# chriscoey/Hypatia.jl

Measured on AMD Instinct MI355X. Metric: IPM iterations/sec (+ ms per KKT solve): dense n=5000, PosSemidefTri side 200 (Float64, QRCholDense + CombinedStepper), higher is better.
Workload: dtype f64

## Files before the change

hypatia.jl_amd/csrc/capi.hip:

```cpp
#include <unistd.h>
#include "../../include/hypatia_hip.h"
#include "syssolver.hpp"
#include <chrono>
#include <cstring>

using namespace hyp;

struct hyp_ctx { Ctx c; hyp_ctx(int d) : c(d) {} };
struct hyp_cone { hyp_ctx* ctx; Cone* cone; };
struct hyp_sys { hyp_ctx* ctx; SysSolver* s; };
struct hyp_symindef { hyp_ctx* ctx; SymIndefSys* s; };
struct hyp_comm { hyp_ctx* ctx; void* nccl; int nranks, rank; };
namespace hyp {
struct QrcpFact;
QrcpFact* qrcp_create(Ctx& c, int m, int n, const double* hA, int lda, const double* hb);
void qrcp_get(QrcpFact* f, int* jpvt, double* R, double* rdiag, double* qtb);
void qrcp_apply_q(QrcpFact* f, bool trans, double* hx);
void qrcp_destroy(QrcpFact* f);
}
struct hyp_qrcp { hyp_ctx* ctx; hyp::QrcpFact* f; };

namespace hyp {
void rccl_allreduce_inplace(void* comm, double* d_buf, long count, int op, hipStream_t st);
void rccl_unique_id(char* out128);
// ... 488 lines not shown
  sys->ctx->c.sync();
  sys->ctx->c.timers[6] += now_s() - t0;
  API_END(sys->ctx)
}
int hyp_sys_lhs_export_dev(hyp_sys* sys, void* dst_device) {
  API_BEGIN
  Ctx& c = sys->ctx->c;
  c.d2d(dst_device, sys->s->lhs.p, (size_t)sys->s->nmp * sys->s->nmp * sizeof(double));
  c.sync();
  API_END(sys->ctx)
}
int hyp_sys_lhs_import_dev(hyp_sys* sys, const void* src_device) {
  API_BEGIN
  Ctx& c = sys->ctx->c;
  c.d2d(sys->s->lhs.p, src_device, (size_t)sys->s->nmp * sys->s->nmp * sizeof(double));
  c.sync();
  API_END(sys->ctx)
}
int hyp_sys_set_lhs(hyp_sys* sys, const double* in) {
  API_BEGIN
  Ctx& c = sys->ctx->c;
  c.h2d(sys->s->lhs.p, in, (size_t)sys->s->nmp * sys->s->nmp * sizeof(double));
  c.sync();
  API_END(sys->ctx)
}
int hyp_sys_potrs(hyp_sys* sys, double* x) {
  API_BEGIN
  Ctx& c = sys->ctx->c;
  SysSolver* s = sys->s;
  HYP_REQUIRE(s->fact_ok, "potrs: no valid factorization");
  c.h2d(s->tmpn.p, x, (size_t)s->nmp * sizeof(double));
  s->potrs(s->tmpn.d());
  c.d2h(x, s->tmpn.p, (size_t)s->nmp * sizeof(double));
  c.sync();
  API_END(sys->ctx)
}
int hyp_sys_solve3(hyp_sys* sys, double* sol_vec, const double* rhs_vec) {
// ... 686 lines not shown
```

hypatia.jl_amd/csrc/directions_multi.hip:

```cpp
#include <cstring>
#include "syssolver.hpp"
#include <chrono>

namespace hyp {

void seg_dots(Ctx& c, int B, int len, const double* a, const double* b, int off, int stride, double* out);
constexpr int MR = 2;

template <int NR, int TPB, int U>
__global__ __launch_bounds__(TPB) void gemv_t_multi_kernel(int m, double alpha, const double* __restrict__ A, long lda,
                                                           const double* __restrict__ X, long ldx, double beta, double* __restrict__ Y,
                                                           long ldy) {
  constexpr int NW = TPB / 64;
  __shared__ double red[NR][NW];
  const int col = blockIdx.x;
  const double* a = A + (long)col * lda;
  double s[NR][2 * U];
#pragma unroll
  for (int r = 0; r < NR; ++r)
#pragma unroll
    for (int u = 0; u < 2 * U; ++u) s[r][u] = 0.0;
  int i = 0;
  typedef double d2_t __attribute__((ext_vector_type(2)));
  const bool wide = (((uintptr_t)a | (uintptr_t)X | ((uintptr_t)ldx * sizeof(double))) & 15) == 0;
// ... 1386 lines not shown
  const auto t0 = std::chrono::steady_clock::now();
  const double tau = h_point[it], kap = h_point[ik];
  m_rhs.ensure((size_t)(MR + 1) * dv * d);
  v_tmp.ensure((size_t)MR * dv * d);
  const bool resident = resident_flow;
  if (!resident) {
    if (nmp > 0) update_lhs_fact(info, used_fallback);
    if (use_sqrt_out)
      for (size_t k = 0; k < cones.size(); ++k) use_sqrt_out[k] = use_sqrt[k];
    if (*info != 0) { ctx.sync(); return; }
    step_directions_rest(false, tau, kap, tau_residual, mu, max_ref_steps, res_norm_cutoff, min_impr_tol, h_dirs, res_norms, n_solves,
                         h_sol_const, hs_const, hs_dirs, false, nullptr, nullptr);
    last_update_lhs_s = last_rest_update_lhs_s + std::chrono::duration<double>(t_rest0 - t0).count();
    return;
  }
  assemble_lhs();
  factor_lhs_begin();
  if (upload_after) {
    hs_point = ctx.stage_host((size_t)dv + 2 * (size_t)it + 2 * (size_t)MR * dv);
    hs_res = hs_point + dv;
    hs_const = hs_res + it;
    hs_dirs = hs_const + it;
    upload(ctx.stream);
  }
  if (upload_late) {
    hs_point = ctx.stage_host((size_t)dv + 2 * (size_t)it + 2 * (size_t)MR * dv);
    hs_res = hs_point + dv;
    hs_const = hs_res + it;
    hs_dirs = hs_const + it;
    HYP_CHECK(hipStreamWaitEvent(ctx.stream2, up_ev0, 0));
    upload(ctx.stream2);
// ... 149 lines not shown
```

hypatia.jl_amd/csrc/gemm_f64.hpp:

```cpp
#pragma once
#include <hip/hip_runtime.h>
#include <stdint.h>

namespace hyp {

typedef double d4_t __attribute__((ext_vector_type(4)));

enum GemmTri : int {
  GEMM_FULL = 0,
  GEMM_UPPER = 1,
  GEMM_UPPER_RECT = 2,
};

enum GemmKRange : int {
  KR_ALL = 0,
  KR_LE_M = 1,
  KR_GE_M = 2,
  KR_LE_N = 3,
  KR_GE_N = 4,
};

struct GemmArgs {
  int M, N, K;
  const double* A; long lda; long strideA;
// ... 4 lines not shown
  int krange;
  int batch;
  int tiles_m, tiles_n;
  int cm_blk; long cm_stride;
  int tile_hint;
  int epi;
  int tag;
  int hiprio;
  int tri_off;
  int splitk_req;
  int splitk; int kchunk; double* part; long part_ld; long part_stride;
  int vec2;
  const int* tile_map;
  int splitk_base, tail_q, tail_first, tail_chunk;
  int* tile_cnt;
};

struct GemmScratch {
  double* splitk_ws = nullptr;
  size_t splitk_ws_bytes = 0;
  int* tile_map = nullptr;
  int tile_map_T = -1;
  int* tile_cnt = nullptr;
  long tile_cnt_n = 0;
  struct TrapMap { int tiles_m = 0, tiles_n = 0, tri_off = 0; long nblk = 0; int* map = nullptr; unsigned long used = 0; };
  TrapMap trap[16];
  unsigned long trap_clock = 0;
  void release() {
    for (TrapMap& t : trap) { if (t.map) (void)hipFree(t.map); t = TrapMap(); }
    if (splitk_ws) (void)hipFree(splitk_ws);
    if (tile_map) (void)hipFree(tile_map);
    if (tile_cnt) (void)hipFree(tile_cnt);
    splitk_ws = nullptr; splitk_ws_bytes = 0; tile_map = nullptr; tile_map_T = -1; tile_cnt = nullptr; tile_cnt_n = 0;
  }
};

hipError_t gemm_f64_launch(hipStream_t st, bool transa, GemmArgs a, GemmScratch* scratch = nullptr);
hipError_t schur_syrk_cols(hipStream_t st, GemmArgs a, int c0, int c1, GemmScratch* scratch);
hipError_t schur_syrk_edge(hipStream_t st, const GemmArgs& a, int* N0);

}
```

hypatia.jl_amd/csrc/gemm_f64_kernel.hpp:

```cpp
#pragma once
#include "gemm_f64.hpp"
#include <vector>

namespace hyp {

#ifdef HYP_GEMM_PROBE
__device__ unsigned long long gemm_probe_acc[8];
#define GEMM_PROBE_T(x) const unsigned long long x = __builtin_amdgcn_s_memtime()
#else
#define GEMM_PROBE_T(x)
#endif

constexpr int BK = 16, LDS_S = BK + 2;
typedef const volatile double __attribute__((address_space(3))) lds_cv_f64;
constexpr int GEMM_THREADS = 256;

__device__ __forceinline__ void upper_tile_from_linear(int idx, int& tm, int& tn) {
  int t = (int)((sqrt(8.0 * (double)idx + 1.0) - 1.0) * 0.5);
  while ((long)(t + 1) * (t + 2) / 2 <= idx) ++t;
  while ((long)t * (t + 1) / 2 > idx) --t;
  tn = t;
  tm = idx - t * (t + 1) / 2;
}

// ... 317 lines not shown
                                     double alpha, double beta, double* __restrict__ C, long ldc, int S_extra, int tail_first,
                                     const int* __restrict__ tile_rank, int T, long part_batch, long strideC) {
  const int m = blockIdx.x * blockDim.x + threadIdx.x;
  const int n = blockIdx.y;
  if (m >= M || (upper && m > n + tri_off)) return;
  part += (long)blockIdx.z * part_batch;
  C += (long)blockIdx.z * strideC;
  double s = 0.0;
  for (int z = 0; z < S; ++z) s += part[(long)z * part_stride + (long)n * part_ld + m];
  if (S_extra > 0 && tile_rank[(m >> 7) + (n >> 7) * T] >= tail_first)
    for (int z = S; z < S + S_extra; ++z) s += part[(long)z * part_stride + (long)n * part_ld + m];
  double* cp = C + (long)n * ldc + m;
  *cp = alpha * s + (beta != 0.0 ? beta * (*cp) : 0.0);
}

static const int* upper_tile_map(GemmScratch& gs, int T, long nblk) {
  if (gs.tile_map_T == T) return gs.tile_map;
  std::vector<int> logical;
  logical.reserve(2 * nblk);
  const int ST = 8, nst = (T + ST - 1) / ST;
  for (int J = 0; J < nst; ++J)
    for (int I = 0; I <= J; ++I)
      for (int j = 0; j < ST; ++j)
        for (int i = 0; i < ST; ++i) {
          const int tm = I * ST + i, tn = J * ST + j;
          if (tm < T && tn < T && tm <= tn) { logical.push_back(tm); logical.push_back(tn); }
        }
  std::vector<int> hw(2 * nblk + (size_t)T * T, -1);
  const long q = nblk / 8, r = nblk % 8;
  for (long b = 0; b < nblk; ++b) {
// ... 39 lines not shown
    hw[2 * b] = logical[2 * L];
    hw[2 * b + 1] = logical[2 * L + 1];
    hw[2 * nblk + hw[2 * b] + (size_t)hw[2 * b + 1] * tiles_m] = (int)b;
  }
  if (slot->map) { (void)hipDeviceSynchronize(); (void)hipFree(slot->map); }
  *slot = GemmScratch::TrapMap();
  int* d = nullptr;
  if (hipMalloc((void**)&d, hw.size() * sizeof(int)) != hipSuccess) return nullptr;
  if (hipMemcpy(d, hw.data(), hw.size() * sizeof(int), hipMemcpyHostToDevice) != hipSuccess) { (void)hipFree(d); return nullptr; }
  slot->map = d; slot->tiles_m = tiles_m; slot->tiles_n = tiles_n; slot->tri_off = tri_off; slot->nblk = nblk; slot->used = ++gs.trap_clock;
  *nblk_out = nblk;
  return d;
}

template <int CB, int R>
__global__ __launch_bounds__(256) void syrk_edge_kernel(int K, int N, int N0, int e0, int r, const double* __restrict__ A, long lda, double alpha,
                                                        double beta, double* __restrict__ C, long ldc) {
  typedef double d2_t __attribute__((ext_vector_type(2)));
  __shared__ double red[CB][R][4];
  const int i0 = blockIdx.x * CB;
  const double* a[CB];
  const double* x[R];
#pragma unroll
  for (int c = 0; c < CB; ++c) a[c] = A + (long)min(i0 + c, N - 1) * lda;
#pragma unroll
  for (int e = 0; e < R; ++e) x[e] = A + (long)min(N0 + e0 + e, N - 1) * lda;
  constexpr int NS = (CB * R <= 32) ? 2 : 1;
  double s[CB][R][NS];
#pragma unroll
  for (int c = 0; c < CB; ++c)
#pragma unroll
    for (int e = 0; e < R; ++e)
#pragma unroll
      for (int h = 0; h < NS; ++h) s[c][e][h] = 0.0;
  const int nfull = K / 512;
// ... 28 lines not shown
#pragma unroll
    for (int e = 0; e < R; ++e) {
      double t = (NS == 2) ? s[c][e][0] + s[c][e][NS - 1] : s[c][e][0];
#pragma unroll
      for (int off = 32; off > 0; off >>= 1) t += __shfl_down(t, off);
      if ((threadIdx.x & 63) == 0) red[c][e][threadIdx.x >> 6] = t;
    }
  __syncthreads();
  if (threadIdx.x < CB * R) {
    const int c = threadIdx.x / R, e = threadIdx.x % R;
    const int i = i0 + c, col = N0 + e0 + e;
    if (i < N && e0 + e < r && i <= col) {
      const double t = (red[c][e][0] + red[c][e][1]) + (red[c][e][2] + red[c][e][3]);
      double* dst = C + (long)col * ldc + i;
      *dst = alpha * t + (beta != 0.0 ? beta * (*dst) : 0.0);
    }
  }
}

static bool syrk_edge_ok(const GemmArgs& a) {
  static const bool edge_on = [] { const char* e = getenv("HYP_SYRK_EDGE"); return !(e && atoi(e) == 0); }();
  return edge_on && ((uintptr_t)a.A % 16 == 0) && (a.lda % 2 == 0);
}
static hipError_t syrk_edge_launch(hipStream_t st, const GemmArgs& a, int N0, int r) {
  static const int cb_env = [] { const char* e = getenv("HYP_SYRK_EDGE_CB"); return e ? atoi(e) : 8; }();
  const int cb = cb_env;
  for (int e0 = 0; e0 < r; e0 += 8) {
    if (cb == 8) hipLaunchKernelGGL((syrk_edge_kernel<8, 8>), dim3((a.N + 7) / 8), dim3(256), 0, st, a.K, a.N, N0, e0, r, a.A, a.lda, a.alpha, a.beta, a.C, a.ldc);
    else hipLaunchKernelGGL((syrk_edge_kernel<4, 8>), dim3((a.N + 3) / 4), dim3(256), 0, st, a.K, a.N, N0, e0, r, a.A, a.lda, a.alpha, a.beta, a.C, a.ldc);
  }
  return hipGetLastError();
}

hipError_t gemm_f64_launch(hipStream_t st, bool transa, GemmArgs a, GemmScratch* gs) {
  if (a.M <= 0 || a.N <= 0 || a.batch <= 0) return hipSuccess;
  if (a.tag == 1 && transa && a.tri == GEMM_UPPER && a.A == a.B && a.lda == a.ldb && a.batch == 1 && a.epi == 0 &&
      a.krange == KR_ALL && a.M == a.N && a.N >= 1024 && a.N % 128 != 0 && a.N % 128 <= 32 && a.K >= 4096) {
    const int r = a.N % 128, N0 = a.N - r;
    GemmArgs m = a;
    m.M = m.N = N0;
    hipError_t e = gemm_f64_launch(st, transa, m, gs);
    if (e != hipSuccess) return e;
    GemmArgs s = a;
    s.tag = 0; s.M = a.N; s.N = r;
    s.B = a.A + (long)N0 * a.lda;
    s.C = a.C + (long)N0 * a.ldc;
    s.tri = GEMM_UPPER_RECT; s.tri_off = N0;
    s.tile_hint = 64; s.splitk_req = 8;
    if (syrk_edge_ok(a)) return syrk_edge_launch(st, a, N0, r);
    return gemm_f64_launch(st, transa, s, gs);
  }
  const long t128 = (long)((a.M + 127) / 128) * ((a.N + 127) / 128) * a.batch;
  const bool small = (a.tile_hint == 64) || (a.tile_hint == 0 && t128 < 192);
  const int BT = small ? 64 : 128;
  a.tiles_m = (a.M + BT - 1) / BT;
  a.tiles_n = (a.N + BT - 1) / BT;
  long nblk;
  const int* trap_map = nullptr;
  static const bool trap_on = [] { const char* e = getenv("HYP_GEMM_TRAP_MAP"); return !(e && atoi(e) == 0); }();
  if (a.tri == GEMM_UPPER) {
    int T = a.tiles_n;
    nblk = (long)T * (T + 1) / 2;
  } else {
    nblk = (long)a.tiles_m * a.tiles_n;
    if (trap_on && gs && a.tag == 1 && transa && a.tri == GEMM_UPPER_RECT && !small && a.batch == 1 && a.epi == 0 && a.krange == KR_ALL && nblk >= 64) {
// ... 85 lines not shown
      gs->tile_cnt = nullptr; gs->tile_cnt_n = 0;
      if (hipMalloc((void**)&gs->tile_cnt, (size_t)nblk * sizeof(int)) == hipSuccess && hipMemset(gs->tile_cnt, 0, (size_t)nblk * sizeof(int)) == hipSuccess)
        gs->tile_cnt_n = nblk;
    }
    if (gs->tile_cnt_n >= nblk) a.tile_cnt = gs->tile_cnt;
  }
  if (a.tag == 1 && transa && !small) {
    hipLaunchKernelGGL((gemm_f64_kernel<true, 4, 1>), grid, dim3(GEMM_THREADS), 0, st, a);
  } else if (transa) {
    if (small) hipLaunchKernelGGL((gemm_f64_kernel<true, 2, 0>), grid, dim3(GEMM_THREADS), 0, st, a);
    else hipLaunchKernelGGL((gemm_f64_kernel<true, 4, 0>), grid, dim3(GEMM_THREADS), 0, st, a);
  } else {
    if (small) hipLaunchKernelGGL((gemm_f64_kernel<false, 2, 0>), grid, dim3(GEMM_THREADS), 0, st, a);
    else hipLaunchKernelGGL((gemm_f64_kernel<false, 4, 0>), grid, dim3(GEMM_THREADS), 0, st, a);
  }
  if (a.splitk > 1 && a.tile_cnt == nullptr)
    hipLaunchKernelGGL(splitk_reduce_kernel, dim3((a.M + 255) / 256, a.N, a.batch), dim3(256), 0, st, a.M, a.N, a.tri != GEMM_FULL ? 1 : 0, a.tri_off,
                       a.splitk_base, a.part, a.part_ld, a.part_stride, a.alpha, a.beta, a.C, a.ldc, a.tail_q - 1, a.tail_first,
                       a.tile_map ? a.tile_map + 2 * nblk : nullptr, trap_map ? a.tiles_m : a.tiles_n, (long)a.splitk * a.part_stride, a.strideC);
  return hipGetLastError();
}

hipError_t schur_syrk_cols(hipStream_t st, GemmArgs a, int c0, int c1, GemmScratch* gs) {
  static const int s_env = [] { const char* e = getenv("HYP_CHOL_SPLIT_S"); return e ? atoi(e) : 0; }();
  if (c0 == 0) {
    GemmArgs l = a;
    l.M = l.N = c1;
    if (s_env > 0) l.splitk_req = s_env;
    return gemm_f64_launch(st, true, l, gs);
  }
  const int N = a.N;
  int r = N % 128, N0 = N - r;
  if (!(r > 0 && r <= 32 && a.K >= 4096 && syrk_edge_ok(a))) { r = 0; N0 = N; }
  GemmArgs t = a;
  t.M = N0; t.N = N0 - c0;
  t.B = a.A + (long)c0 * a.lda;
  t.C = a.C + (long)c0 * a.ldc;
  t.tri = GEMM_UPPER_RECT; t.tri_off = c0;
  if (t.N > 0) {
    const long tm = (t.M + 127) / 128, tn = (t.N + 127) / 128, tc0 = c0 / 128;
    long real = 0;
    for (long j = 0; j < tn; ++j) real += std::min(tm, tc0 + j + 1);
    int S = 1;
    double best = 1e30;
    const double eps = ((double)t.M * t.N * 4.6e-12) / (2.6e-7 * a.K);
    for (int q = 1; q <= 8; ++q) {
      if (a.K / q < 1024) break;
      const double cost = (double)((real * q + 511) / 512) / q + (q > 1 ? q * eps : 0.0);
      if (cost < best - 1e-9) { best = cost; S = q; }
    }
    if (s_env > 0) S = s_env;
    t.splitk_req = S;
    hipError_t e = gemm_f64_launch(st, true, t, gs);
    if (e != hipSuccess) return e;
  }
  if (r > 0) return syrk_edge_launch(st, a, N0, r);
  return hipSuccess;
}

hipError_t schur_syrk_edge(hipStream_t st, const GemmArgs& a, int* N0) {
  const int r = a.N % 128;
  *N0 = a.N;
  if (!(r > 0 && r <= 32 && a.N >= 1024 && a.K >= 4096 && a.M == a.N && syrk_edge_ok(a))) return hipSuccess;
  *N0 = a.N - r;
  return syrk_edge_launch(st, a, *N0, r);
}

}
// ... 1 lines not shown
```

hypatia.jl_amd/csrc/syssolver.hip:

```cpp
#include <cstring>
#include "syssolver.hpp"
#include <chrono>

namespace hyp {

__global__ void increase_diag_kernel(int n, double* A, long lda) {
  const int j = blockIdx.x * blockDim.x + threadIdx.x;
  if (j < n) {
    const double d = A[(long)j * lda + j];
    A[(long)j * lda + j] = (1.0 + 1e-5) * fmax(d, 1000 * 2.220446049250313e-16);
  }
}

SysSolver::SysSolver(Ctx& c, int n_, int p_, int q_, const std::vector<Cone*>& cs) : ctx(c), n(n_), p(p_), q(q_), nmp(n_ - p_), cones(cs) {
  HYP_REQUIRE(n >= 0 && p >= 0 && q >= 0 && p <= n, "sys: sizes");
  offs.assign(cones.size() + 1, 0);
  for (size_t k = 0; k < cones.size(); ++k) offs[k + 1] = offs[k] + cones[k]->dim;
  HYP_REQUIRE(offs.back() == q, "sys: cone dimensions do not sum to q");
  use_sqrt.assign(cones.size(), 0);
  make_psd_runs();
  const size_t d = sizeof(double);
  G.alloc((size_t)q * n * d);
  if (p > 0) {
    GQ1.alloc((size_t)q * p * d);
// ... 12 lines not shown
  tmpn.alloc((size_t)std::max(n, 1) * d);
  Gx.alloc((size_t)std::max(q, 1) * d);
  HGx.alloc((size_t)std::max(q, 1) * d);
  tmpq.alloc((size_t)std::max(q, 1) * d);
  sol.alloc((size_t)(n + p + q + 1) * d);
  rhs.alloc((size_t)(n + p + q + 1) * d);
}

SysSolver::~SysSolver() {
  if (const char* e = getenv("HYP_RP_PREFETCH_STATS"))
    if (e[0] == '1') fprintf(stderr, "[residual_products prefetch] handed out %ld, recomputed %ld\n", rp_pre_hits, rp_pre_misses);
  if (const char* e = getenv("HYP_SHP_PRELAUNCH_STATS"))
    if (e[0] == '1') fprintf(stderr, "[sqrt_hess_prod prelaunch] used %ld, not used %ld\n", shp_used, shp_unused);
  if (const char* e = getenv("HYP_CHOL_SPLIT_STATS"))
    if (e[0] == '1') fprintf(stderr, "[chol split] %ld factorizations in two column groups\n", chol_split_count);
  if (rp_pre_host) (void)hipHostFree(rp_pre_host);
  for (hipEvent_t e : {rp_pre_ev, plan_ev_fork, plan_ev_done, dirs_copied_ev, up_ev0, up_ev1, split_ev_ready, split_ev_done, ov_ev_fork})
    if (e) (void)hipEventDestroy(e);
}

void SysSolver::make_psd_runs() {
  static const bool on = [] { const char* e = getenv("HYP_PSD_GROUP"); return !(e && e[0] == '0'); }();
  if (!on) return;
  size_t k = 0;
  while (k < cones.size()) {
    PsdCone* pk = (cones[k]->kind == CONE_PSD) ? static_cast<PsdCone*>(cones[k]) : nullptr;
    size_t e = k + 1;
    if (pk)
      while (e < cones.size() && cones[e]->kind == CONE_PSD && static_cast<PsdCone*>(cones[e])->side == pk->side) ++e;
    const int cnt = (int)(e - k);
// ... 338 lines not shown
void SysSolver::comm_times_flush() {
  for (const CommEv& e : comm_ev_pending) {
    HYP_CHECK(hipEventSynchronize(e.b));
    float ms = 0;
    HYP_CHECK(hipEventElapsedTime(&ms, e.a, e.b));
    comm_ms[e.site] += ms;
    comm_ev_free.push_back(e.a);
    comm_ev_free.push_back(e.b);
  }
  comm_ev_pending.clear();
}

void SysSolver::allreduce_lhs() {
  const bool have = (comm_fn != nullptr || rccl_comm != nullptr);
  if (!have || (ks_world <= 1 && !dist())) return;
  const int kw = ks_world;
  ks_world = 1;
  hipEvent_t ev_whole = nullptr;
  comm_time_begin(14, &ev_whole);
  try {
    const long cnt = (long)nmp * (nmp + 1) / 2;
    lhs_tri.ensure((size_t)cnt * sizeof(double));
    const dim3 grid((nmp + 255) / 256, nmp);
    hipLaunchKernelGGL(tri_pack_kernel, grid, dim3(256), 0, ctx.stream, nmp, lhs.d(), (long)nmp, lhs_tri.d(), 0);
    allreduce_dev(lhs_tri.d(), cnt, 0, 0);
    hipLaunchKernelGGL(tri_pack_kernel, grid, dim3(256), 0, ctx.stream, nmp, lhs.d(), (long)nmp, lhs_tri.d(), 1);
    HYP_CHECK(hipGetLastError());
  } catch (...) {
    ks_world = kw;
    throw;
// ... 200 lines not shown
}

void SysSolver::block_hess_prod_vec(double* d_out, const double* d_in) {
  for (size_t k = 0; k < cones.size(); ++k) {
    Cone* ck = cones[k];
    if (const int used = run_hess_prod(k, d_out + offs[k], q, d_in + offs[k], q, 1)) { k += used - 1; continue; }
    if (ck->use_dual_barrier) ck->inv_hess_prod(d_out + offs[k], q, d_in + offs[k], q, 1);
    else ck->hess_prod(d_out + offs[k], q, d_in + offs[k], q, 1);
  }
}

void SysSolver::update_lhs_fact(int* info, int* used_fallback) {
  *info = 0;
  *used_fallback = 0;
  if (nmp == 0) return;
  assemble_lhs();
  factor_lhs(info, used_fallback);
}

static bool force_bk_env();

void SysSolver::prelaunch_sqrt_hess() {
  static const bool on = [] { const char* e = getenv("HYP_SHP_PRELAUNCH"); return e && e[0] == '1'; }();
  shp_prelaunched = false;
  if (!on || shp_wasted >= 2 || nmp <= 0 || p != 0 || dist() || ks_world > 1 || !dirs_resident() || force_bk_env() ||
      ctx.stream != ctx.stream_primary)
    return;
  {
    const char* ff = getenv("HYP_FORCE_FACT_FAIL");
    if (ff && ff[0] && ff[0] != '0') return;
  }
// ... 6 lines not shown
  if (!all_sqrt) return;
  const double* gq2 = GQ2();
  HYP_CHECK(hipEventRecord(ctx.ev[0], ctx.stream));
  int idx = 0;
  for (size_t k = 0; k < cones.size(); ++k) {
    Cone* ck = cones[k];
    if (ck->use_dual_barrier) ck->inv_sqrt_hess_prod(HGQ2.d() + idx, q, gq2 + offs[k], q, nmp);
    else ck->sqrt_hess_prod(HGQ2.d() + idx, q, gq2 + offs[k], q, nmp);
    idx += ck->dim;
  }
  HYP_CHECK(hipEventRecord(ctx.ev[1], ctx.stream));
  shp_prelaunched = true;
  shp_epoch = ctx.cone_epoch;
}

void SysSolver::assemble_lhs() {
  if (split_unjoined) {
    HYP_CHECK(hipStreamWaitEvent(ctx.stream, split_ev_done, 0));
    split_unjoined = false;
  }
  chol_split_n1 = 0;
  const bool pre = shp_prelaunched && shp_epoch == ctx.cone_epoch && nmp > 0 && !dist() && ks_world == 1;
  if (shp_prelaunched) {
    if (pre) { shp_wasted = 0; ++shp_used; }
    else { ++shp_wasted; ++shp_unused; }
  }
  shp_prelaunched = false;
  if (!pre) group_inverses();
  if (nmp == 0) return;
  const double* gq2 = GQ2();
  if (!pre)
// ... 31 lines not shown
    if (!pre) HYP_CHECK(hipEventRecord(ctx.ev[1], ctx.stream));
    GemmArgs s{};
    long r0 = 0, r1 = idx;
    if (ks_world > 1) {
      const long per = (((long)idx + ks_world - 1) / ks_world + 15) / 16 * 16;
      r0 = std::min<long>((long)idx, per * ks_rank);
      r1 = std::min<long>((long)idx, r0 + per);
    }
    if (use_ov && assemble_lhs_overlapped(r0, r1, ov_groups)) {
      HYP_CHECK(hipEventRecord(ctx.ev[2], ctx.stream));
      ctx.kstat[4] += 1;
      return;
    }
    s.M = nmp; s.N = nmp; s.K = (int)(r1 - r0); s.A = HGQ2.d() + r0; s.lda = q; s.B = HGQ2.d() + r0; s.ldb = q; s.C = lhs.d(); s.ldc = nmp;
    s.alpha = 1; s.beta = 0; s.tri = GEMM_UPPER; s.krange = KR_ALL; s.batch = 1; s.tag = 1;
    {
      bool all_sqrt = true;
      for (int v : use_sqrt) all_sqrt &= (v != 0);
      const int n1 = chol_split_point(nmp, s.K);
      if (n1 > 0 && all_sqrt && !dist() && ks_world == 1 && !force_bk_env() && ctx.stream == ctx.stream_primary) {
        if (!split_ev_ready) {
          HYP_CHECK(hipEventCreateWithFlags(&split_ev_ready, hipEventDisableTiming));
          HYP_CHECK(hipEventCreateWithFlags(&split_ev_done, hipEventDisableTiming));
        }
        schur_split_begin(ctx, nmp, s.K, s.A, q, lhs.d(), lhs_fact.d(), n1, d_info.i(), ctx.lane(2).s, split_ev_ready, split_ev_done);
        chol_split_n1 = n1;
        split_unjoined = true;
        HYP_CHECK(hipEventRecord(ctx.ev[2], ctx.stream));
        ctx.kstat[4] += 1;
        return;
      }
    }
    gemm(ctx, true, s);
    HYP_CHECK(hipEventRecord(ctx.ev[2], ctx.stream));
    ctx.kstat[4] += 1;
  } else {
    ctx.zero(lhs.p, (size_t)nmp * nmp * sizeof(double));
  }
  for (size_t k = 0; k < cones.size(); ++k) {
    if (use_sqrt[k]) continue;
    Cone* ck = cones[k];
    double* prod_k = HGQ2.d() + offs[k];
    if (ck->use_dual_barrier) ck->inv_hess_prod(prod_k, q, gq2 + offs[k], q, nmp);
    else ck->hess_prod(prod_k, q, gq2 + offs[k], q, nmp);
    long r0 = 0, r1 = ck->dim;
    if (ks_world > 1) {
      const long per = (((long)ck->dim + ks_world - 1) / ks_world + 15) / 16 * 16;
      r0 = std::min<long>((long)ck->dim, per * ks_rank);
      r1 = std::min<long>((long)ck->dim, r0 + per);
    }
    if (r1 <= r0) continue;
    GemmArgs g{};
    g.M = nmp; g.N = nmp; g.K = (int)(r1 - r0); g.A = gq2 + offs[k] + r0; g.lda = q; g.B = prod_k + r0; g.ldb = q; g.C = lhs.d(); g.ldc = nmp;
    g.alpha = 1; g.beta = 1; g.tri = GEMM_UPPER; g.krange = KR_ALL; g.batch = 1;
    gemm(ctx, true, g);
  }
  allreduce_lhs();
}

static bool force_bk_env() {
  const char* fb = getenv("HYP_FORCE_BK");
  return fb && fb[0] && fb[0] != '0';
}

int SysSolver::chol_split_point(int n, int K) {
  static const int pct = [] { const char* e = getenv("HYP_CHOL_SPLIT"); return e ? atoi(e) : 0; }();
  static const int min_n = [] { const char* e = getenv("HYP_CHOL_SPLIT_MIN_N"); return e ? atoi(e) : 3072; }();
  if (pct <= 0 || n < min_n || K < 4096) return 0;
  int n1 = (int)((long)n * std::min(pct, 95) / 100) / 128 * 128;
  return potrf_split_ok(n, n1) ? n1 : 0;
}

void SysSolver::factor_lhs_begin() {
  if (nmp == 0 || force_bk_env()) return;
  use_bk = false;
  if (chol_split_n1 > 0) {
    HYP_CHECK(hipEventRecord(ctx.ev[3], ctx.stream));
    schur_split_finish(ctx, nmp, lhs.d(), lhs_fact.d(), chol_split_n1, dinv.d(), d_info.i(), split_ev_done);
    chol_split_n1 = 0;
    split_unjoined = false;
    ++chol_split_count;
  } else {
    ctx.d2d(lhs_fact.p, lhs.p, (size_t)nmp * nmp * sizeof(double));
    HYP_CHECK(hipEventRecord(ctx.ev[3], ctx.stream));
    potrf_upper_batched(ctx, nmp, lhs_fact.d(), nmp, 0, 1, dinv.d(), d_info.i());
  }
  HYP_CHECK(hipEventRecord(ctx.ev[4], ctx.stream));
  ctx.d2h(ctx.h_info + Ctx::H_INFO_FACT, d_info.p, sizeof(int));
  tri.invalidate();
  if (ctx.trsv_plan_sb(nmp) <= 0) return;
  static const bool plan_lane = [] { const char* e = getenv("HYP_PLAN_LANE"); return e && e[0] == '1'; }();
  if (plan_lane && Ctx::max_lanes() >= 3 && ctx.stream == ctx.stream_primary) {
    if (!plan_ev_fork) {
      HYP_CHECK(hipEventCreateWithFlags(&plan_ev_fork, hipEventDisableTiming));
      HYP_CHECK(hipEventCreateWithFlags(&plan_ev_done, hipEventDisableTiming));
    }
    HYP_CHECK(hipEventRecord(plan_ev_fork, ctx.stream));
    {
// ... 25 lines not shown
void SysSolver::factor_lhs_end(int* info, int* used_fallback, bool times_later) {
  *info = 0;
  *used_fallback = 0;
  if (nmp == 0) return;
  const bool force_bk = force_bk_env();
  use_bk = false;
  join_plan();
  if (!force_bk) {
    *info = ctx.h_info[Ctx::H_INFO_FACT];
    if (!times_later) factor_lhs_times();
  }
  if (force_bk || *info != 0) {
    use_bk = true;
    *used_fallback = 1;
    const int chol_info = force_bk ? 0 : *info;
    ctx.d2d(lhs_fact.p, lhs.p, (size_t)nmp * nmp * sizeof(double));
    *info = bk_after_failed_cholesky(ctx, bk, nmp, lhs_fact.d(), nmp, dinv.d(), d_info.i(), chol_info, lhs.d(), nmp);
    if (*info != 0) {
      *used_fallback = 2;
      ctx.d2d(lhs_fact.p, lhs.p, (size_t)nmp * nmp * sizeof(double));
      hipLaunchKernelGGL(increase_diag_kernel, dim3((nmp + 255) / 256), dim3(256), 0, ctx.stream, nmp, lhs_fact.d(), (long)nmp);
      *info = bk.factor(ctx, nmp, lhs_fact.d(), nmp, dinv.d());
    }
  }
  {
    const char* ff = getenv("HYP_FORCE_FACT_FAIL");
    if (ff && ff[0] && ff[0] != '0') *info = 1;
  }
  fact_ok = (*info == 0);
  if (use_bk || !fact_ok) tri.invalidate();
// ... 1284 lines not shown
```

hypatia.jl_amd/csrc/syssolver.hpp:

```cpp
#pragma once
#include <chrono>
#include "cones.hpp"

namespace hyp {

void dev_sub_absmax(Ctx& c, int n, double* a, const double* b, double* d_out);
void dev_sub_absmax_cols(Ctx& c, int n, int nr, double* a, const double* b, long ld, double* d_out, double* work);

struct SysSolver {
  Ctx& ctx;
  int n, p, q, nmp;
  std::vector<Cone*> cones;
  std::vector<int> offs;
  DBuf G;
  DBuf GQ1;
  DBuf GQ2s;
  DBuf Qm;
  DBuf Rinv;
  DBuf HGQ2;
  DBuf lhs;
  DBuf lhs_tri;
  DBuf lhs_fact, dinv, d_info;
  TriSolvePlan tri;
  DBuf QpbxGHbz, Gx, HGx, GQ1x, HGQ1x, tmpn, sol, rhs, tmpq;
// ... 10 lines not shown
  void run_dder3(const PsdRun& r, const double* d_dir, double* d_out);
  void run_prox_launch(const PsdRun& r, double irtmu, double* d_out);
  DBuf prox_scal;
  BKFact bk;
  bool use_bk = false;
  DBuf bk_work;

  SysSolver(Ctx& c, int n_, int p_, int q_, const std::vector<Cone*>& cs);
  ~SysSolver();
  SysSolver(const SysSolver&) = delete;
  SysSolver& operator=(const SysSolver&) = delete;
  const double* GQ2() const { return p == 0 ? G.d() : GQ2s.d(); }
  void load(const double* hG, const double* hGQ1, const double* hGQ2, const double* hQ, const double* hR);
  void block_hess_prod_vec(double* d_out, const double* d_in);
  void update_lhs_fact(int* info, int* used_fallback);
  void assemble_lhs();
  void factor_lhs(int* info, int* used_fallback);
  void prelaunch_sqrt_hess();
  bool shp_prelaunched = false;
  unsigned long shp_epoch = 0;
  int shp_wasted = 0;
  long shp_used = 0, shp_unused = 0;
  int chol_split_point(int n, int K);
  int chol_split_n1 = 0;
  long chol_split_count = 0;
  bool split_unjoined = false;
  hipEvent_t split_ev_ready = nullptr, split_ev_done = nullptr;
  hipEvent_t ov_ev_fork = nullptr;
  void factor_lhs_begin();
  void factor_lhs_end(int* info, int* used_fallback, bool times_later = false);
  hipEvent_t plan_ev_fork = nullptr, plan_ev_done = nullptr;
// ... 163 lines not shown
```

Measured before the change: 58.50.

## Write Schur product directly into factor buffer and fuse edge SYRK into split-K finish

The split-K reduction for the upper-triangular Schur complement SYRK now writes its result to both lhs and lhs_fact, so the full nmp×nmp device-to-device copy before Cholesky can be skipped when the lower part of lhs_fact is known to be valid. The edge-column SYRK for the N%128 remainder is folded into the same finish kernel launch instead of running as separate kernels. State flags track when lhs_fact is filled and invalidate that on imports, allreduce, split factorization or fallback paths. This adds a second store stream in the reduce and more bookkeeping that must stay correct across code paths.

```diff
diff --git a/hypatia.jl_amd/csrc/capi.hip b/hypatia.jl_amd/csrc/capi.hip
--- a/hypatia.jl_amd/csrc/capi.hip
+++ b/hypatia.jl_amd/csrc/capi.hip
@@ -526,6 +526,7 @@
   API_BEGIN
   Ctx& c = sys->ctx->c;
   c.d2d(sys->s->lhs.p, src_device, (size_t)sys->s->nmp * sys->s->nmp * sizeof(double));
+  sys->s->lhs_fact_filled = false; sys->s->lhs_fact_lower_ok = false;
   c.sync();
   API_END(sys->ctx)
 }
@@ -533,6 +534,7 @@
   API_BEGIN
   Ctx& c = sys->ctx->c;
   c.h2d(sys->s->lhs.p, in, (size_t)sys->s->nmp * sys->s->nmp * sizeof(double));
+  sys->s->lhs_fact_filled = false; sys->s->lhs_fact_lower_ok = false;
   c.sync();
   API_END(sys->ctx)
 }
diff --git a/hypatia.jl_amd/csrc/directions_multi.hip b/hypatia.jl_amd/csrc/directions_multi.hip
--- a/hypatia.jl_amd/csrc/directions_multi.hip
+++ b/hypatia.jl_amd/csrc/directions_multi.hip
@@ -1424,7 +1424,7 @@
     last_update_lhs_s = last_rest_update_lhs_s + std::chrono::duration<double>(t_rest0 - t0).count();
     return;
   }
-  assemble_lhs();
+  assemble_lhs(true);
   factor_lhs_begin();
   if (upload_after) {
     hs_point = ctx.stage_host((size_t)dv + 2 * (size_t)it + 2 * (size_t)MR * dv);
diff --git a/hypatia.jl_amd/csrc/gemm_f64.hpp b/hypatia.jl_amd/csrc/gemm_f64.hpp
--- a/hypatia.jl_amd/csrc/gemm_f64.hpp
+++ b/hypatia.jl_amd/csrc/gemm_f64.hpp
@@ -42,6 +42,7 @@
   const int* tile_map;
   int splitk_base, tail_q, tail_first, tail_chunk;
   int* tile_cnt;
+  double* C2; long ldc2;
 };
 
 struct GemmScratch {
@@ -54,6 +55,7 @@
   struct TrapMap { int tiles_m = 0, tiles_n = 0, tri_off = 0; long nblk = 0; int* map = nullptr; unsigned long used = 0; };
   TrapMap trap[16];
   unsigned long trap_clock = 0;
+  bool c2_done = false;
   void release() {
     for (TrapMap& t : trap) { if (t.map) (void)hipFree(t.map); t = TrapMap(); }
     if (splitk_ws) (void)hipFree(splitk_ws);
diff --git a/hypatia.jl_amd/csrc/gemm_f64_kernel.hpp b/hypatia.jl_amd/csrc/gemm_f64_kernel.hpp
--- a/hypatia.jl_amd/csrc/gemm_f64_kernel.hpp
+++ b/hypatia.jl_amd/csrc/gemm_f64_kernel.hpp
@@ -355,6 +355,81 @@
   *cp = alpha * s + (beta != 0.0 ? beta * (*cp) : 0.0);
 }
 
+struct SchurFinishArgs {
+  int M, N, tri_off, S_extra, tail_first, T;
+  const double* part; long part_ld, part_stride;
+  const int* tile_rank;
+  double alpha, beta;
+  double* C; long ldc;
+  double* C2; long ldc2;
+  int n_edge, K, r;
+  const double* A; long lda;
+};
+
+template <int S, int ROWS>
+__device__ __forceinline__ void schur_reduce_body(const SchurFinishArgs& p, int b) {
+  typedef double d2_t __attribute__((ext_vector_type(2)));
+  constexpr int TPC = 128 / ROWS;
+  constexpr int CPP = 256 / TPC;
+  constexpr int U = 2;
+  int tm, tn;
+  upper_tile_from_linear(b >> 3, tm, tn);
+  const int extra = (p.S_extra > 0 && p.tile_rank[tm + tn * p.T] >= p.tail_first) ? p.S_extra : 0;
+  const int m = tm * 128 + ROWS * ((int)threadIdx.x % TPC);
+  const int nb = tn * 128 + (b & 7) * 16 + (int)threadIdx.x / TPC;
+#pragma unroll 1
+  for (int c = 0; c < 16; c += U * CPP) {
+    bool ok[U][ROWS];
+    long off[U];
+    double v[U][S][ROWS], cold[U][ROWS];
+#pragma unroll
+    for (int u = 0; u < U; ++u) {
+      const int n = nb + c + u * CPP;
+#pragma unroll
+      for (int h = 0; h < ROWS; ++h) ok[u][h] = (n < p.N) && (m + h < p.M) && (m + h <= n + p.tri_off);
+      off[u] = ok[u][0] ? (long)n * p.part_ld + m : 0;
+#pragma unroll
+      for (int z = 0; z < S; ++z) {
+        const double* src = p.part + (long)z * p.part_stride + off[u];
+        if (ROWS == 2) {
+          const d2_t t = *reinterpret_cast<const d2_t*>(src);
+          v[u][z][0] = t.x; v[u][z][ROWS - 1] = t.y;
+        } else {
+          v[u][z][0] = *src;
+        }
+      }
+      if (p.beta != 0.0) {
+        const double* cp = p.C + (ok[u][0] ? (long)n * p.ldc + m : 0);
+#pragma unroll
+        for (int h = 0; h < ROWS; ++h) cold[u][h] = cp[h];
+      }
+    }
+#pragma unroll
+    for (int u = 0; u < U; ++u) {
+      const int n = nb + c + u * CPP;
+      double res[ROWS];
+#pragma unroll
+      for (int h = 0; h < ROWS; ++h) {
+        double s = 0.0;
+#pragma unroll
+        for (int z = 0; z < S; ++z) s += v[u][z][h];
+        for (int z = S; z < S + extra; ++z) s += p.part[(long)z * p.part_stride + off[u] + h];
+        res[h] = p.alpha * s + (p.beta != 0.0 ? p.beta * cold[u][h] : 0.0);
+      }
+      if (!ok[u][0]) continue;
+      double* cp = p.C + (long)n * p.ldc + m;
+      double* cp2 = p.C2 ? p.C2 + (long)n * p.ldc2 + m : nullptr;
+      if (ROWS == 2 && ok[u][ROWS - 1]) {
+        *reinterpret_cast<d2_t*>(cp) = (d2_t){res[0], res[ROWS - 1]};
+        if (cp2) *reinterpret_cast<d2_t*>(cp2) = (d2_t){res[0], res[ROWS - 1]};
+      } else {
+        *cp = res[0];
+        if (cp2) *cp2 = res[0];
+      }
+    }
+  }
+}
+
 static const int* upper_tile_map(GemmScratch& gs, int T, long nblk) {
   if (gs.tile_map_T == T) return gs.tile_map;
   std::vector<int> logical;
@@ -424,11 +499,10 @@
 }
 
 template <int CB, int R>
-__global__ __launch_bounds__(256) void syrk_edge_kernel(int K, int N, int N0, int e0, int r, const double* __restrict__ A, long lda, double alpha,
-                                                        double beta, double* __restrict__ C, long ldc) {
+__device__ __forceinline__ void syrk_edge_body(int i0, int K, int N, int N0, int e0, int r, const double* __restrict__ A, long lda, double alpha,
+                                               double beta, double* __restrict__ C, long ldc, double* __restrict__ C2, long ldc2) {
   typedef double d2_t __attribute__((ext_vector_type(2)));
   __shared__ double red[CB][R][4];
-  const int i0 = blockIdx.x * CB;
   const double* a[CB];
   const double* x[R];
 #pragma unroll
@@ -487,41 +561,94 @@
       const double t = (red[c][e][0] + red[c][e][1]) + (red[c][e][2] + red[c][e][3]);
       double* dst = C + (long)col * ldc + i;
       *dst = alpha * t + (beta != 0.0 ? beta * (*dst) : 0.0);
-    }
-  }
+      if (C2) C2[(long)col * ldc2 + i] = *dst;
+    }
+  }
+}
+
+template <int CB, int R>
+__global__ __launch_bounds__(256) void syrk_edge_kernel(int K, int N, int N0, int e0, int r, const double* __restrict__ A, long lda, double alpha,
+                                                        double beta, double* __restrict__ C, long ldc, double* __restrict__ C2, long ldc2) {
+  syrk_edge_body<CB, R>(blockIdx.x * CB, K, N, N0, e0, r, A, lda, alpha, beta, C, ldc, C2, ldc2);
+}
+
+template <int S, int ROWS, bool EDGE>
+__global__ __launch_bounds__(256) void schur_finish_kernel(SchurFinishArgs p) {
+  if (EDGE && (int)blockIdx.x < p.n_edge) {
+    const int nb = (p.N + p.r + 7) / 8;
+    syrk_edge_body<8, 8>(((int)blockIdx.x % nb) * 8, p.K, p.N + p.r, p.N, ((int)blockIdx.x / nb) * 8, p.r, p.A, p.lda, p.alpha, p.beta, p.C, p.ldc,
+                         p.C2, p.ldc2);
+    return;
+  }
+  schur_reduce_body<S, ROWS>(p, (int)blockIdx.x - p.n_edge);
 }
 
 static bool syrk_edge_ok(const GemmArgs& a) {
   static const bool edge_on = [] { const char* e = getenv("HYP_SYRK_EDGE"); return !(e && atoi(e) == 0); }();
   return edge_on && ((uintptr_t)a.A % 16 == 0) && (a.lda % 2 == 0);
 }
-static hipError_t syrk_edge_launch(hipStream_t st, const GemmArgs& a, int N0, int r) {
+static int syrk_edge_cb() {
   static const int cb_env = [] { const char* e = getenv("HYP_SYRK_EDGE_CB"); return e ? atoi(e) : 8; }();
-  const int cb = cb_env;
+  return cb_env;
+}
+static hipError_t syrk_edge_launch(hipStream_t st, const GemmArgs& a, int N0, int r, double* C2 = nullptr, long ldc2 = 0) {
+  const int cb = syrk_edge_cb();
   for (int e0 = 0; e0 < r; e0 += 8) {
-    if (cb == 8) hipLaunchKernelGGL((syrk_edge_kernel<8, 8>), dim3((a.N + 7) / 8), dim3(256), 0, st, a.K, a.N, N0, e0, r, a.A, a.lda, a.alpha, a.beta, a.C, a.ldc);
-    else hipLaunchKernelGGL((syrk_edge_kernel<4, 8>), dim3((a.N + 3) / 4), dim3(256), 0, st, a.K, a.N, N0, e0, r, a.A, a.lda, a.alpha, a.beta, a.C, a.ldc);
+    if (cb == 8)
+      hipLaunchKernelGGL((syrk_edge_kernel<8, 8>), dim3((a.N + 7) / 8), dim3(256), 0, st, a.K, a.N, N0, e0, r, a.A, a.lda, a.alpha, a.beta, a.C, a.ldc, C2, ldc2);
+    else
+      hipLaunchKernelGGL((syrk_edge_kernel<4, 8>), dim3((a.N + 3) / 4), dim3(256), 0, st, a.K, a.N, N0, e0, r, a.A, a.lda, a.alpha, a.beta, a.C, a.ldc, C2, ldc2);
   }
   return hipGetLastError();
 }
 
-hipError_t gemm_f64_launch(hipStream_t st, bool transa, GemmArgs a, GemmScratch* gs) {
+static int schur_finish_mode() {
+  static const int mode = [] { const char* e = getenv("HYP_SCHUR_FINISH"); return e ? atoi(e) : 1; }();
+  return mode;
+}
+
+template <int ROWS, bool EDGE>
+static void schur_finish_launch(hipStream_t st, int S, long nblocks, const SchurFinishArgs& f) {
+  const dim3 grid((unsigned)nblocks), blk(256);
+  switch (S) {
+    case 1: hipLaunchKernelGGL((schur_finish_kernel<1, ROWS, EDGE>), grid, blk, 0, st, f); break;
+    case 2: hipLaunchKernelGGL((schur_finish_kernel<2, ROWS, EDGE>), grid, blk, 0, st, f); break;
+    case 3: hipLaunchKernelGGL((schur_finish_kernel<3, ROWS, EDGE>), grid, blk, 0, st, f); break;
+    case 4: hipLaunchKernelGGL((schur_finish_kernel<4, ROWS, EDGE>), grid, blk, 0, st, f); break;
+    case 5: hipLaunchKernelGGL((schur_finish_kernel<5, ROWS, EDGE>), grid, blk, 0, st, f); break;
+    case 6: hipLaunchKernelGGL((schur_finish_kernel<6, ROWS, EDGE>), grid, blk, 0, st, f); break;
+    case 7: hipLaunchKernelGGL((schur_finish_kernel<7, ROWS, EDGE>), grid, blk, 0, st, f); break;
+    default: hipLaunchKernelGGL((schur_finish_kernel<8, ROWS, EDGE>), grid, blk, 0, st, f); break;
+  }
+}
+
+static hipError_t gemm_f64_launch_impl(hipStream_t st, bool transa, GemmArgs a, GemmScratch* gs, int edge_r, int* fin) {
+  if (fin) *fin = 0;
   if (a.M <= 0 || a.N <= 0 || a.batch <= 0) return hipSuccess;
+  const int fin_mode = fin ? schur_finish_mode() : 0;
+  if (fin_mode == 0 || fin_mode == 3) { a.C2 = nullptr; a.ldc2 = 0; }
   if (a.tag == 1 && transa && a.tri == GEMM_UPPER && a.A == a.B && a.lda == a.ldb && a.batch == 1 && a.epi == 0 &&
       a.krange == KR_ALL && a.M == a.N && a.N >= 1024 && a.N % 128 != 0 && a.N % 128 <= 32 && a.K >= 4096) {
     const int r = a.N % 128, N0 = a.N - r;
     GemmArgs m = a;
     m.M = m.N = N0;
-    hipError_t e = gemm_f64_launch(st, transa, m, gs);
+    const bool edge_in_finish = (fin_mode == 1 || fin_mode == 3) && syrk_edge_ok(a) && syrk_edge_cb() == 8;
+    int f = 0;
+    hipError_t e = gemm_f64_launch_impl(st, transa, m, gs, edge_in_finish ? r : 0, fin ? &f : nullptr);
     if (e != hipSuccess) return e;
+    if (f & 2) { *fin = 1; return hipSuccess; }
     GemmArgs s = a;
     s.tag = 0; s.M = a.N; s.N = r;
     s.B = a.A + (long)N0 * a.lda;
     s.C = a.C + (long)N0 * a.ldc;
     s.tri = GEMM_UPPER_RECT; s.tri_off = N0;
     s.tile_hint = 64; s.splitk_req = 8;
-    if (syrk_edge_ok(a)) return syrk_edge_launch(st, a, N0, r);
-    return gemm_f64_launch(st, transa, s, gs);
+    s.C2 = nullptr; s.ldc2 = 0;
+    if (syrk_edge_ok(a)) {
+      if (f & 1) *fin = 1;
+      return syrk_edge_launch(st, a, N0, r, (f & 1) ? a.C2 : nullptr, a.ldc2);
+    }
+    return gemm_f64_launch_impl(st, transa, s, gs, 0, nullptr);
   }
   const long t128 = (long)((a.M + 127) / 128) * ((a.N + 127) / 128) * a.batch;
   const bool small = (a.tile_hint == 64) || (a.tile_hint == 0 && t128 < 192);
@@ -637,11 +764,35 @@
     if (small) hipLaunchKernelGGL((gemm_f64_kernel<false, 2, 0>), grid, dim3(GEMM_THREADS), 0, st, a);
     else hipLaunchKernelGGL((gemm_f64_kernel<false, 4, 0>), grid, dim3(GEMM_THREADS), 0, st, a);
   }
-  if (a.splitk > 1 && a.tile_cnt == nullptr)
+  if (fin_mode != 0 && a.splitk > 1 && a.tile_cnt == nullptr && a.tag == 1 && transa && a.tri == GEMM_UPPER && a.M == a.N && a.batch == 1 &&
+      a.splitk_base <= 8) {
+    SchurFinishArgs f{};
+    f.M = a.M; f.N = a.N; f.tri_off = a.tri_off; f.S_extra = a.tail_q - 1; f.tail_first = a.tail_first; f.T = a.tiles_n;
+    f.part = a.part; f.part_ld = a.part_ld; f.part_stride = a.part_stride;
+    f.tile_rank = a.tile_map ? a.tile_map + 2 * nblk : nullptr;
+    f.alpha = a.alpha; f.beta = a.beta; f.C = a.C; f.ldc = a.ldc; f.C2 = a.C2; f.ldc2 = a.ldc2;
+    f.n_edge = edge_r > 0 ? ((a.N + edge_r + 7) / 8) * ((edge_r + 7) / 8) : 0;
+    f.K = a.K; f.r = edge_r; f.A = a.A; f.lda = a.lda;
+    const long T128 = (a.N + 127) / 128;
+    const long nblocks = f.n_edge + 8 * (T128 * (T128 + 1) / 2);
+    const bool rows2 = a.M % 2 == 0 && (uintptr_t)a.C % 16 == 0 && a.ldc % 2 == 0 && (a.C2 == nullptr || ((uintptr_t)a.C2 % 16 == 0 && a.ldc2 % 2 == 0));
+    if (rows2 && f.n_edge > 0) schur_finish_launch<2, true>(st, a.splitk_base, nblocks, f);
+    else if (rows2) schur_finish_launch<2, false>(st, a.splitk_base, nblocks, f);
+    else if (f.n_edge > 0) schur_finish_launch<1, true>(st, a.splitk_base, nblocks, f);
+    else schur_finish_launch<1, false>(st, a.splitk_base, nblocks, f);
+    *fin = 1 | (edge_r > 0 ? 2 : 0);
+  } else if (a.splitk > 1 && a.tile_cnt == nullptr)
     hipLaunchKernelGGL(splitk_reduce_kernel, dim3((a.M + 255) / 256, a.N, a.batch), dim3(256), 0, st, a.M, a.N, a.tri != GEMM_FULL ? 1 : 0, a.tri_off,
                        a.splitk_base, a.part, a.part_ld, a.part_stride, a.alpha, a.beta, a.C, a.ldc, a.tail_q - 1, a.tail_first,
                        a.tile_map ? a.tile_map + 2 * nblk : nullptr, trap_map ? a.tiles_m : a.tiles_n, (long)a.splitk * a.part_stride, a.strideC);
   return hipGetLastError();
+}
+
+hipError_t gemm_f64_launch(hipStream_t st, bool transa, GemmArgs a, GemmScratch* gs) {
+  int fin = 0;
+  const hipError_t e = gemm_f64_launch_impl(st, transa, a, gs, 0, &fin);
+  if (gs && a.C2) gs->c2_done = (e == hipSuccess) && (fin & 1) && schur_finish_mode() != 3;
+  return e;
 }
 
 hipError_t schur_syrk_cols(hipStream_t st, GemmArgs a, int c0, int c1, GemmScratch* gs) {
@@ -650,7 +801,7 @@
     GemmArgs l = a;
     l.M = l.N = c1;
     if (s_env > 0) l.splitk_req = s_env;
-    return gemm_f64_launch(st, true, l, gs);
+    return gemm_f64_launch_impl(st, true, l, gs, 0, nullptr);
   }
   const int N = a.N;
   int r = N % 128, N0 = N - r;
@@ -674,7 +825,7 @@
     }
     if (s_env > 0) S = s_env;
     t.splitk_req = S;
-    hipError_t e = gemm_f64_launch(st, true, t, gs);
+    hipError_t e = gemm_f64_launch_impl(st, true, t, gs, 0, nullptr);
     if (e != hipSuccess) return e;
   }
   if (r > 0) return syrk_edge_launch(st, a, N0, r);
diff --git a/hypatia.jl_amd/csrc/syssolver.hip b/hypatia.jl_amd/csrc/syssolver.hip
--- a/hypatia.jl_amd/csrc/syssolver.hip
+++ b/hypatia.jl_amd/csrc/syssolver.hip
@@ -50,6 +50,8 @@
     if (e[0] == '1') fprintf(stderr, "[sqrt_hess_prod prelaunch] used %ld, not used %ld\n", shp_used, shp_unused);
   if (const char* e = getenv("HYP_CHOL_SPLIT_STATS"))
     if (e[0] == '1') fprintf(stderr, "[chol split] %ld factorizations in two column groups\n", chol_split_count);
+  if (const char* e = getenv("HYP_SCHUR_FINISH_STATS"))
+    if (e[0] == '1') fprintf(stderr, "[schur finish] lhs_fact written by the product %ld times, copied %ld times\n", lhs_fact_fills, lhs_fact_copies);
   if (rp_pre_host) (void)hipHostFree(rp_pre_host);
   for (hipEvent_t e : {rp_pre_ev, plan_ev_fork, plan_ev_done, dirs_copied_ev, up_ev0, up_ev1, split_ev_ready, split_ev_done, ov_ev_fork})
     if (e) (void)hipEventDestroy(e);
@@ -418,6 +420,7 @@
 void SysSolver::allreduce_lhs() {
   const bool have = (comm_fn != nullptr || rccl_comm != nullptr);
   if (!have || (ks_world <= 1 && !dist())) return;
+  lhs_fact_filled = false;
   const int kw = ks_world;
   ks_world = 1;
   hipEvent_t ev_whole = nullptr;
@@ -648,7 +651,7 @@
   *info = 0;
   *used_fallback = 0;
   if (nmp == 0) return;
-  assemble_lhs();
+  assemble_lhs(true);
   factor_lhs(info, used_fallback);
 }
 
@@ -685,7 +688,8 @@
   shp_epoch = ctx.cone_epoch;
 }
 
-void SysSolver::assemble_lhs() {
+void SysSolver::assemble_lhs(bool factor_follows) {
+  lhs_fact_filled = false;
   if (split_unjoined) {
     HYP_CHECK(hipStreamWaitEvent(ctx.stream, split_ev_done, 0));
     split_unjoined = false;
@@ -747,9 +751,9 @@
     }
     s.M = nmp; s.N = nmp; s.K = (int)(r1 - r0); s.A = HGQ2.d() + r0; s.lda = q; s.B = HGQ2.d() + r0; s.ldb = q; s.C = lhs.d(); s.ldc = nmp;
     s.alpha = 1; s.beta = 0; s.tri = GEMM_UPPER; s.krange = KR_ALL; s.batch = 1; s.tag = 1;
+    bool all_sqrt = true;
+    for (int v : use_sqrt) all_sqrt &= (v != 0);
     {
-      bool all_sqrt = true;
-      for (int v : use_sqrt) all_sqrt &= (v != 0);
       const int n1 = chol_split_point(nmp, s.K);
       if (n1 > 0 && all_sqrt && !dist() && ks_world == 1 && !force_bk_env() && ctx.stream == ctx.stream_primary) {
         if (!split_ev_ready) {
@@ -764,7 +768,10 @@
         return;
       }
     }
+    const bool fill_fact = factor_follows && all_sqrt && !dist() && ks_world == 1 && !force_bk_env() && lhs_fact_lower_ok;
+    if (fill_fact) { s.C2 = lhs_fact.d(); s.ldc2 = nmp; }
     gemm(ctx, true, s);
+    if (fill_fact && ctx.gemm_scratch.c2_done) { lhs_fact_filled = true; lhs_fact_stream = ctx.stream; }
     HYP_CHECK(hipEventRecord(ctx.ev[2], ctx.stream));
     ctx.kstat[4] += 1;
   } else {
@@ -783,6 +790,7 @@
       r1 = std::min<long>((long)ck->dim, r0 + per);
     }
     if (r1 <= r0) continue;
+    lhs_fact_filled = false;
     GemmArgs g{};
     g.M = nmp; g.N = nmp; g.K = (int)(r1 - r0); g.A = gq2 + offs[k] + r0; g.lda = q; g.B = prod_k + r0; g.ldb = q; g.C = lhs.d(); g.ldc = nmp;
     g.alpha = 1; g.beta = 1; g.tri = GEMM_UPPER; g.krange = KR_ALL; g.batch = 1;
@@ -813,8 +821,16 @@
     chol_split_n1 = 0;
     split_unjoined = false;
     ++chol_split_count;
+    lhs_fact_lower_ok = false;
   } else {
-    ctx.d2d(lhs_fact.p, lhs.p, (size_t)nmp * nmp * sizeof(double));
+    if (!(lhs_fact_filled && lhs_fact_stream == ctx.stream)) {
+      ctx.d2d(lhs_fact.p, lhs.p, (size_t)nmp * nmp * sizeof(double));
+      lhs_fact_lower_ok = true;
+      ++lhs_fact_copies;
+    } else {
+      ++lhs_fact_fills;
+    }
+    lhs_fact_filled = false;
     HYP_CHECK(hipEventRecord(ctx.ev[3], ctx.stream));
     potrf_upper_batched(ctx, nmp, lhs_fact.d(), nmp, 0, 1, dinv.d(), d_info.i());
   }
@@ -870,6 +886,7 @@
     use_bk = true;
     *used_fallback = 1;
     const int chol_info = force_bk ? 0 : *info;
+    lhs_fact_lower_ok = false;
     ctx.d2d(lhs_fact.p, lhs.p, (size_t)nmp * nmp * sizeof(double));
     *info = bk_after_failed_cholesky(ctx, bk, nmp, lhs_fact.d(), nmp, dinv.d(), d_info.i(), chol_info, lhs.d(), nmp);
     if (*info != 0) {
diff --git a/hypatia.jl_amd/csrc/syssolver.hpp b/hypatia.jl_amd/csrc/syssolver.hpp
--- a/hypatia.jl_amd/csrc/syssolver.hpp
+++ b/hypatia.jl_amd/csrc/syssolver.hpp
@@ -48,7 +48,11 @@
   void load(const double* hG, const double* hGQ1, const double* hGQ2, const double* hQ, const double* hR);
   void block_hess_prod_vec(double* d_out, const double* d_in);
   void update_lhs_fact(int* info, int* used_fallback);
-  void assemble_lhs();
+  void assemble_lhs(bool factor_follows = false);
+  bool lhs_fact_filled = false;
+  bool lhs_fact_lower_ok = false;
+  hipStream_t lhs_fact_stream = nullptr;
+  long lhs_fact_fills = 0, lhs_fact_copies = 0;
   void factor_lhs(int* info, int* used_fallback);
   void prelaunch_sqrt_hess();
   bool shp_prelaunched = false;
```

New measurement: 59.35, median of 6. 1.01x the previous value.
